# proger/haloop

Hardware: AMD Instinct MI355X
Metric: utterances/sec, LSTM-CTC training step (fwd + CTC loss + bwd + clip + AdamW) (higher is better)
Workload: dtype bf16 (dense operands rounded to bf16, 1 MFMA per product, fp32 accumulate; fp32 state, CTC, optimizer and master weights); 1 GPU; LC-2x1024: conv(80->128,k5,s4) + 2-layer LSTM H=1024 + Linear(1024->32) + CTC, 80 frames x 80 mels, vocab 32, targets 5-10 symbols, dropout 0.2; batch_per_gpu=64, global_batch=64, frames=80, mels=80, parallelism=dp1, hip_graph=False, math=bf16

## Files before the change

haloop_amd/_lib.py:

```python
import ctypes as C
import os

_HERE = os.path.dirname(os.path.abspath(__file__))
LIB_PATH = os.path.join(_HERE, 'csrc', 'libhalo.so')

HALO_ABI_VERSION = 21
HALO_GPT_SAMPLE_STREAM = 0x47505453
HALO_MLM_STREAM = 0x4D4C4D31
HALO_GEMM_RELU = 1
HALO_GEMM_GELU = 2
HALO_GEMM_ACCUM = 4
HALO_GEMM_GELU_ERF = 8
HALO_CTC_FULL_LATTICE = 1
HALO_CTC_FINITE_MIN = 2
HALO_CTC_NO_LEAD_BLANK_LOOP = 4
HALO_CTC_WRAP_SKIP = 8
HALO_STREAM_SUBSAMPLE = 1
HALO_STREAM_CLASSIFIER = 2
HALO_STREAM_LSTM_LAYER0 = 16
HALO_SUMSQ_PARTS = 1024
HALO_MATH_F32 = 0
HALO_MATH_BF16X3 = 1
HALO_MATH_BF16 = 2

# ... 174 lines not shown
    'halo_mlm_batch_u16': (_i, [_vp, _l, _vp, _i, _i, _f, _l, _l, _l, _u64, _u32, _vp, _vp, _vp]),
    'halo_target_rows': (_i, [_vp, _i, _l, _i, _i, _vp, _vp, _vp, _vp, _vp]),
    'halo_gather_rows': (_i, [_vp, _vp, _i, _i, _i, _vp, _vp]),
    'halo_scatter_rows': (_i, [_vp, _vp, _vp, _i, _i, _i, _i, _vp, _vp, _vp]),
    'halo_scale_add': (_i, [_vp, _vp, _f, _f, _sz, _vp]),
    'halo_cast_f32_bf16': (_i, [_vp, _vp, _sz, _vp]),
    'halo_cast_bf16_f32': (_i, [_vp, _vp, _f, _sz, _vp]),
    'halo_scale_add_guarded': (_i, [_vp, _vp, _f, _f, _sz, _vp, _vp]),
    'halo_clip_coef_step': (_i, [_vp, _i, _f, _vp, _vp, _vp, _vp]),
    'halo_adamw_ranges_dev': (_i, [_vp, _vp, _vp, _vp, _i, _vp, _vp, _vp, _vp, _f, _vp, _f, _f, _f, _vp, _vp, _vp]),
    'halo_ctx_create': (_vp, []),
    'halo_ctx_destroy': (None, [_vp]),
    'halo_ctx_use': (_i, [_vp]),
    'halo_set_status_word': (_i, [_vp]),
    'halo_debug_mute_workgroup': (_i, [_i]),
    'halo_debug_mfma_clock': (_i, [_vp, _vp, _i, _i, _i, _u32, _vp]),
    'halo_sumsq': (_i, [_vp, _sz, _vp, _vp]),
    'halo_sumsq_ranges': (_i, [_vp, _i, _vp, _vp, _vp, _vp]),
    'halo_pack_ranges_bf16': (_i, [_vp, _i, _vp, _vp, _vp, _vp]),
    'halo_expand_ranges_bf16': (_i, [_vp, _i, _vp, _vp, _i, _i, _vp, _vp]),
    'halo_clip_coef': (_i, [_vp, _i, _f, _vp, _vp, _vp]),
    'halo_adamw_multi_tensor_bytes': (_sz, []),
    'halo_adamw_multi_chunk': (_u32, []),
    'halo_adamw_multi_max_tensors': (_i, []),
    'halo_adamw_multi': (_i, [_vp, _vp, _i, _vp, _i, _f, _f, _f, _f, _i, _vp, _vp]),
    'halo_adamw_ranges': (_i, [_vp, _vp, _vp, _vp, _i, _vp, _vp, _vp, _vp, _f, _f, _f, _f, _i, _vp, _vp]),
    'halo_adamw': (_i, [_vp, _vp, _vp, _vp, _sz, _f, _f, _f, _f, _f, _i, _vp, _vp]),
}

_lib = None
# ... 168 lines not shown
```

haloop_amd/csrc/halo_common.h:

```cpp
#pragma once
#include <hip/hip_runtime.h>
#include <stdint.h>
#include "halo.h"

#define HALO_WAVE 64

#define HALO_CHECK_ARG(cond) \
    do {                     \
        if (!(cond)) return HALO_EINVAL; \
    } while (0)

static inline int halo_launch_status() {
    return hipGetLastError() == hipSuccess ? HALO_OK : HALO_ELAUNCH;
}

typedef float f32x4 __attribute__((ext_vector_type(4)));
typedef float f32x16 __attribute__((ext_vector_type(16)));

struct Philox4 {
    uint32_t v[4];
};

__device__ __forceinline__ Philox4 philox4x32_10(uint32_t c0, uint32_t c1, uint32_t c2, uint32_t c3,
                                                 uint32_t k0, uint32_t k1) {
// ... 31 lines not shown
    d.offset = offset;
    if (p > 0.f) {
        double t = (double)p * 4294967296.0;
        d.threshold = t >= 4294967295.0 ? 0xffffffffu : (uint32_t)t;
        d.scale = 1.0f / (1.0f - p);
    } else {
        d.threshold = 0u;
        d.scale = 1.0f;
    }
    return d;
}

__device__ __forceinline__ float dropout_mult(const DropoutCfg &d, uint64_t e) {
    const uint64_t q = e >> 2;
    const uint32_t off = d.offset + (d.offset_dev ? *d.offset_dev : 0u);
    const Philox4 r = philox4x32_10((uint32_t)q, (uint32_t)(q >> 32), d.stream_id, off, d.k0, d.k1);
    const uint32_t lane = (uint32_t)(e & 3);
    const uint32_t v = lane == 0 ? r.v[0] : lane == 1 ? r.v[1] : lane == 2 ? r.v[2] : r.v[3];
    return v >= d.threshold ? d.scale : 0.f;
}

__device__ __forceinline__ f32x4 dropout_mult4(const DropoutCfg &d, uint64_t e) {
    const uint64_t q = e >> 2;
    const uint32_t off = d.offset + (d.offset_dev ? *d.offset_dev : 0u);
    const Philox4 r = philox4x32_10((uint32_t)q, (uint32_t)(q >> 32), d.stream_id, off, d.k0, d.k1);
    f32x4 m;
    m[0] = r.v[0] >= d.threshold ? d.scale : 0.f;
    m[1] = r.v[1] >= d.threshold ? d.scale : 0.f;
    m[2] = r.v[2] >= d.threshold ? d.scale : 0.f;
    m[3] = r.v[3] >= d.threshold ? d.scale : 0.f;
// ... 64 lines not shown
```

haloop_amd/csrc/halo_internal.h:

```cpp
#pragma once
#include <hip/hip_runtime.h>
#include <stddef.h>
#include "halo_common.h"
#include "dyn_lds.h"
#include "small_jobs.h"

int halo_transpose(const float *in, float *out, int rows, int cols, hipStream_t st);
int halo_fill(float *p, size_t n, float v, hipStream_t st);
int halo_colsum2(const float *x, int rows, int cols, int ld, float *out, float *out2, hipStream_t st);

size_t halo_tiled_image_bytes(int R, int K);
int halo_prep_tiles(const float *src, int R, int K, int ld, int src_transposed, void *image, hipStream_t st);
int halo_prep_pair(const float *src, int R, int C, int ld, void *image_rm, void *image_tr, hipStream_t st);
struct HaloPrepJob {
    int kind;
    const float *src;
    int R, K, ld;
    void *image, *image_tr;
};
int halo_prep_jobs(const HaloPrepJob *jobs, int n, hipStream_t st);
int halo_gemm_bf16x3_tiled(const void *Aimg, const void *Bimg, int M, int N, int K, float *C, int ldc,
                           const float *bias1, const float *bias2, int relu, const DropoutCfg *drop, hipStream_t st);
int halo_gemm_bf16x3_tiled_slices(const void *Aimg, const void *Bimg, int M, int N, int K, float *slab, int want, int *slices, hipStream_t st);
bool halo_defer_small_job(const HaloSmallJob &job);
// ... 17 lines not shown
    unsigned grad_sumsq_cover = 0;
    int defer_small_jobs = 0;
    HaloSmallJobs small_jobs = {};
    int lstm_dx_slabs = 1;
    int lstm_dx_slabs_left = 1;
    int lstm_expect_backward = 1;
    const float *packT_reserve = nullptr, *packT_w[3] = {nullptr, nullptr, nullptr};
    const float *bwdflags_reserve = nullptr;
    const float *fwdT_src[2] = {nullptr, nullptr};
    const float *fwdT_reserve = nullptr;
    const float *emitT_reserve = nullptr;
    uint64_t lstm_weights_stamp = 0, packF_stamp = 0;
    const float *packF_reserve = nullptr, *packF_w[3] = {nullptr, nullptr, nullptr};
    int packF_dims[5] = {0, 0, 0, 0, 0};
    int mute_block = -1;
};
HaloCtx &halo_ctx_cur();
int halo_cu_count();
int halo_gemm_bf16x3_tiled_nsplit(const void *Aimg, const void *Bimg, int M, int N, int K, float *C, int ldc, int n_split, float *C2, int ldc2,
                                  hipStream_t st);
int halo_gemm_bf16x3_tiled_nsplit_carry(const void *Aimg, const void *Bimg, int M, int N, int K, float *C, int ldc, int n_split, float *C2, int ldc2,
                                        const void *rA, const void *rB, int rM, int rN, int rK, float *rslab, int want, int *slices,
                                        float *sumsq_part, int *sumsq_parts, hipStream_t st);
struct HaloG256Problem {
    const void *A, *B;
    int M, N, K;
    float *C; int ldc;
    int n_split; float *C2; int ldc2;
    int kslices; long slab_stride;
    float *sumsq;
// ... 15 lines not shown
```

haloop_amd/csrc/lstm_persist.h:

```cpp
#pragma once
#include <hip/hip_runtime.h>
#include <stdlib.h>
#include <type_traits>
#include "halo_common.h"
#include "halo_internal.h"

constexpr int PERSIST_FLAG_HEADER = 16;
constexpr int PERSIST_MAX_BLOCKS = 256;
constexpr int PERSIST_REPLICAS = 8;
constexpr int PERSIST_REPLICA_WORDS = 1024;
constexpr size_t PERSIST_FLAG_BYTES = (size_t)PERSIST_REPLICAS * PERSIST_REPLICA_WORDS * sizeof(unsigned);

struct PersistFwd {
    const char *wp;
    char *hp;
    float *gates;
    float *h;
    float *c;
    float *y;
    long y_stride_t, y_stride_b;
    int y_mode;
    DropoutCfg drop;
    unsigned *flags;
    unsigned *status;
// ... 39 lines not shown
    const char *wp0, *wp1, *wpi;
    char *hp0, *hp1;
    char *xp;
    float *gates0, *h0, *c0;
    float *gates1, *h1, *c1;
    const float *b_ih1, *b_hh1;
    float *ydrop;
    float *y;
    long y_stride_t, y_stride_b;
    int y_mode;
    DropoutCfg drop;
    char *img_hT0, *img_hT1, *img_xT1;
    unsigned *flags;
    unsigned *status;
    int mute;
    unsigned long long *stamps;
    int poll_mode, replica_shift, nap;
    int T, B, H;
    int bt0, nbt;
    unsigned epoch0;
};

struct Persist2Bwd {
    const char *wpT0, *wpT1, *wpTi;
    char *dgp0, *dgp1;
    float *gates0, *gates1;
    const float *c0, *c1;
    float *dc0, *dc1;
    const float *dy;
    long dy_stride_t, dy_stride_b;
    int dy_relu;
    const float *dhinit0, *dcinit0, *dhinit1, *dcinit1;
    DropoutCfg drop;
    unsigned *flags;
    unsigned *abort_word;
// ... 25 lines not shown
    int poll_mode, replica_shift, nap;
};
inline const PersistEnv &halo_persist_env() {
    const auto num = [](const char *name, int dflt) { const char *e = getenv(name); return e ? atoi(e) : dflt; };
    static const PersistEnv env = {num("HALO_PERSIST_POLL", 0), num("HALO_PERSIST_REPLICA_SHIFT", 3), num("HALO_PERSIST_NAP", 2)};
    return env;
}

template <auto Kernel, typename A>
int halo_persist_launch(const A &a0, int blocks, int dyn_lds, hipStream_t st, int poll_mode = 0) {
    static_assert(sizeof(A) <= 4096, "kernel arguments");
    A a = a0;
    a.poll_mode = poll_mode; a.replica_shift = halo_persist_env().replica_shift; a.nap = halo_persist_env().nap;
    a.status = halo_ctx_cur().status;
    if constexpr (std::is_same_v<A, PersistFwd> || std::is_same_v<A, Persist2Fwd>) a.mute = halo_ctx_cur().mute_block;
    if (halo_launch_lds<Kernel>(dim3((unsigned)blocks), dim3(512), dyn_lds, st, a) != HALO_OK) return HALO_ELAUNCH;
    return halo_launch_status();
}
```

haloop_amd/csrc/lstm_persist.hip:

```cpp
#include <stdlib.h>
#include "halo_common.h"
#include "halo_internal.h"
#include "lstm_persist.h"
#include "lstm_persist_dev.h"

namespace {

template <int KBW, bool ONE>
__global__ __launch_bounds__(512, 2) void lstm_persist_fwd_kernel(const PersistFwd p) {
    __shared__ float red[NWAVE][4][256];
    __shared__ __attribute__((aligned(16))) float hbuf[16][16];
    __shared__ int s_abort;
    const int tid = threadIdx.x, lane = tid & 63;
    const int wave = __builtin_amdgcn_readfirstlane(tid >> 6);
    const int H = p.H, B = p.B, T = p.T;
    const int NJ = H / 16, NBT = (B + 15) / 16, nkb = H / 32;
    int jt, bt;
    map_block(blockIdx.x, gridDim.x, NJ, NBT, jt, bt);
    const int j0 = jt * 16;

    bf16x8 wh[4][KBW], wl[4][KBW];
#pragma unroll
    for (int g = 0; g < 4; ++g)
#pragma unroll
// ... 312 lines not shown
            const int g = tid >> 4, j = tid & 15;
            float sum = 0.f;
#pragma unroll
            for (int r = 0; r < 16; ++r) sum += dgbuf[g][r][j];
            p.bias_part[(long)bt * K + (long)g * H + j0 + j] = sum;
        }
    }
}

}

void halo_lstm_persist_enable(int on) { halo_ctx_cur().lstm_persistent = on ? 1 : 0; }
unsigned long long *halo_lstm_persist_stamp_buffer() { return halo_ctx_cur().stamps; }
extern "C" int halo_debug_mute_workgroup(int block) {
    halo_ctx_cur().mute_block = block;
    return HALO_OK;
}
extern "C" int halo_lstm_persist_stamps(void *buf) {
    halo_ctx_cur().stamps = (unsigned long long *)buf;
    return HALO_OK;
}

bool halo_lstm_persist_fits(int T, int B, int H) {
    const long nbt = (B + 15) / 16;
    return (long)(T + 1) * nbt * (4 * H / 32) * 2048 < (1L << 31) && (long)(T + 1) * B * 4 * H < (1L << 31);
}

static bool wide_enabled() {
    static const bool off = getenv("HALO_LSTM_PERSIST32") && atoi(getenv("HALO_LSTM_PERSIST32")) == 0;
    return !off;
// ... 52 lines not shown
```

haloop_amd/csrc/lstm_persist2.hip:

```cpp
#include <stdlib.h>
#include "halo_common.h"
#include "halo_internal.h"
#include "lstm_persist.h"
#include "lstm_persist_dev.h"

namespace {

__device__ __forceinline__ bf16x8 unarm(bf16x8 v) {
    u32x4 w = __builtin_bit_cast(u32x4, v);
    if ((w.x & 0xffffu) == 0xffffu) w.x -= 1u;
    return __builtin_bit_cast(bf16x8, w);
}
template <int N>
__device__ __forceinline__ bool armed_lane(const bf16x8 (&f)[N]) {
    bool a = false;
#pragma unroll
    for (int i = 0; i < N; ++i) a |= (__builtin_bit_cast(u32x4, f[i]).x & 0xffffu) == 0xffffu;
    return a;
}
__device__ __forceinline__ bool rearm_wait(unsigned long long &t0, int pass, int nap) {
    const unsigned long long now = __builtin_amdgcn_s_memrealtime();
    if (pass == 0) t0 = now;
    else if (now - t0 > SPIN_TIMEOUT_TICKS) return false;
    if (nap == 1) __builtin_amdgcn_s_sleep(1);
    else if (nap == 2) __builtin_amdgcn_s_sleep(4);
    else if (nap == 3) __builtin_amdgcn_s_sleep(16);
    return true;
}
__device__ __forceinline__ void stamp_value(unsigned long long *stamps, int T, int step, int point, int lane, unsigned v) {
    if (stamps && lane == 0) stamps[((long)blockIdx.x * T + step) * 16 + point] = v;
}

struct Fwd2Shared {
    float (*red)[4][4][256];
    float (*hbuf)[16][16];
    int *s_abort;
    unsigned *s_published;
};

template <int KBQ, bool DF>
__device__ __forceinline__ void fwd2_layer0_waves(const Persist2Fwd &p, const Fwd2Shared sh, int jt, int bt, int wave, int lane, int u) {
    const int wq = wave & 3;
    const int H = p.H, B = p.B, T = p.T;
    const int NJ = H / 16, NBT = (B + 15) / 16, nkb = H / 32, j0 = jt * 16;
    bf16x8 wr[4][KBQ];
#pragma unroll
    for (int g = 0; g < 4; ++g)
#pragma unroll
        for (int i = 0; i < KBQ; ++i)
            wr[g][i] = *reinterpret_cast<const bf16x8 *>(p.wp0 + (((long)jt * 4 + g) * nkb + wq * KBQ + i) * 2048 + lane * 16);
    const int ci = u >> 4, cj = u & 15;
    const int b = bt * 16 + ci;
    const bool cell = b < B;
    const int BH = B * H;
    const int e0 = b * H + j0 + cj;
    float cst = 0.f, gin[4] = {0.f, 0.f, 0.f, 0.f};
    float dmul = (cell && p.xp) ? dropout_mult(p.drop, (uint64_t)e0) : 1.f;
    if (cell) {
        cst = p.c0[e0];
#pragma unroll
        for (int g = 0; g < 4; ++g) gin[g] = p.gates0[b * 4 * H + g * H + j0 + cj];
    }
    const __amdgpu_buffer_rsrc_t hp0_rsrc = make_rsrc(p.hp0), hp1_rsrc = make_rsrc(p.hp1);
    const __amdgpu_buffer_rsrc_t x_rsrc = p.xp ? make_rsrc(p.xp) : hp0_rsrc;
    const int my_replica = (xcc_id() + p.replica_shift) % PERSIST_REPLICAS;
    const int btl = bt - p.bt0;
    const unsigned *grp_flags = p.flags + my_replica * PERSIST_REPLICA_WORDS + PERSIST_FLAG_HEADER + btl * NJ;
    for (int s = 0; s <= T + 1; ++s) {
        if (wave == 0) stamp(p.stamps, T + 2, s, 0, lane);
        const bool act0 = s < T, act1 = s >= 2;
        if (!DF) {
            bool ok = true;
            if (s > 0 && wave == 1) ok = poll_group(grp_flags, 0, NJ, p.epoch0 + (unsigned)s, lane, p.nap);
            if (!ok && lane == 0) {
                *sh.s_abort = 1;
                raise_abort(p.flags, p.status);
            }
        }
        lds_barrier();
        if (*sh.s_abort) return;
        if (wave == 0) stamp(p.stamps, T + 2, s, 1, lane);
        if (act0) {
            const int img = ((s * NBT + bt) * nkb + wq * KBQ) * 2048;
            bf16x8 ah[KBQ];
            f32x4 acc[4];
            unsigned long long t0 = 0;
            for (int pass = 0;; ++pass) {
#pragma unroll
                for (int i = 0; i < KBQ; ++i) ah[i] = load_sc1_u(hp0_rsrc, lane * 16, img + i * 2048);
                __builtin_amdgcn_sched_barrier(0);
#pragma unroll
                for (int g = 0; g < 4; ++g) acc[g] = f32x4{0.f, 0.f, 0.f, 0.f};
#pragma unroll
                for (int i = 0; i < KBQ; ++i)
#pragma unroll
                    for (int g = 0; g < 4; ++g) acc[g] = __builtin_amdgcn_mfma_f32_16x16x32_bf16(ah[i], wr[g][i], acc[g], 0, 0, 0);
                if (!DF) break;
                if (!__any(armed_lane<KBQ>(ah))) {
                    if (wave == 0) { stamp(p.stamps, T + 2, s, 10, lane); stamp_value(p.stamps, T + 2, s, 11, lane, (unsigned)pass); }
                    break;
                }
                if (!rearm_wait(t0, pass, p.nap)) {
                    if (lane == 0) { *sh.s_abort = 1; raise_abort(p.flags, p.status); }
                    break;
                }
            }
            const int r = lane & 15, q = lane >> 4;
#pragma unroll
            for (int g = 0; g < 4; ++g)
#pragma unroll
                for (int e = 0; e < 4; ++e) sh.red[0][wq][g][(4 * q + e) * 16 + r] = acc[g][e];
        }
        lds_barrier();
        if (DF && *sh.s_abort) return;
        if (wave == 0) stamp(p.stamps, T + 2, s, 2, lane);
        float ig = 0.f, fg = 0.f, gg = 0.f, og = 0.f, h = 0.f, xv = 0.f;
        if (act0) {
            if (cell) {
                float pre[4];
#pragma unroll
                for (int g = 0; g < 4; ++g) {
                    float sum = 0.f;
#pragma unroll
                    for (int k = 0; k < 4; ++k) sum += sh.red[0][k][g][u];
                    pre[g] = sum + gin[g];
                }
                h = persist2_fwd_cell(pre, cst, ig, fg, gg, og);
                if (p.xp) xv = h * dmul;
            }
            sh.hbuf[0][ci][cj] = h;
            if (p.xp) sh.hbuf[1][ci][cj] = xv;
        }
        lds_barrier();
        if (wave == 0) stamp(p.stamps, T + 2, s, 3, lane);
        if ((wave == 3 && act0) || (wave == 2 && act1)) {
            const int sel = lane >> 5, kg = (lane >> 4) & 1, row = lane & 15;
            const float(*src)[16] = wave == 2 ? sh.hbuf[2] : sh.hbuf[sel];
            bf16x8 hi;
#pragma unroll
            for (int e = 0; e < 8; ++e) hi[e] = (__bf16)src[row][kg * 8 + e];
            if (DF) hi = unarm(hi);
            const int within = (jt >> 1) * 2048 + (((jt & 1) * 2 + kg) * 16 + row) * 16;
            const bool store = !DF || (int)blockIdx.x != p.mute;
            if (wave == 3) {
                if (sel == 0 && store) store_sc1(hp0_rsrc, (((s + 1) * NBT + bt) * nkb) * 2048 + within, hi);
                else if (sel == 1 && p.xp && store) store_sc1(x_rsrc, ((s * NBT + bt) * nkb) * 2048 + within, hi);
            } else if (sel == 0 && store) {
                store_sc1(hp1_rsrc, (((s - 1) * NBT + bt) * nkb) * 2048 + within, hi);
            }
            if (DF) {
                stamp(p.stamps, T + 2, s, wave == 3 ? 4 : 5, lane);
            } else {
                asm volatile("s_waitcnt vmcnt(0)" ::: "memory");
                unsigned old = 0;
                if (lane == 0) old = atomicAdd(sh.s_published, 1u);
                old = __builtin_amdgcn_readfirstlane(old);
                const unsigned target = (unsigned)((s + 1 < T ? s + 1 : T) + (s >= 2 ? s - 1 : 0));
                if (old + 1u == target && (int)blockIdx.x != p.mute) publish_epoch(p.flags, btl * NJ + jt, p.epoch0 + (unsigned)(s + 1), lane);
                stamp(p.stamps, T + 2, s, wave == 3 ? 4 : 5, lane);
            }
        } else if (!DF && wave == 3 && !act0 && !act1) {
            publish_epoch(p.flags, btl * NJ + jt, p.epoch0 + (unsigned)(s + 1), lane);
        }
        if (p.img_hT0 && ((wave == 3 && act0) || (wave == 2 && act1))) {
            const int sel = lane >> 5, kg = (lane >> 4) & 1, row = lane & 15;
            const float(*src)[16] = wave == 2 ? sh.hbuf[2] : (sel == 1 && p.xp ? sh.hbuf[1] : sh.hbuf[0]);
            const int tb = wave == 2 ? s - 1 : (sel == 0 ? s + 1 : s);
            char *img = wave == 2 ? (sel == 0 ? p.img_hT1 : nullptr) : (sel == 0 ? p.img_hT0 : p.img_xT1);
            if (img && tb < T) {
                bf16x8 hit;
#pragma unroll
                for (int e = 0; e < 8; ++e) hit[e] = (__bf16)src[kg * 8 + e][row];
                const int grow = j0 + row, kcol = tb * B + bt * 16 + kg * 8;
                const int KT = (T * B + 31) >> 5;
                const long blk = ((long)(grow >> 7) * KT + (kcol >> 5)) * 2;
                const int r = grow & 127, cc = (kcol & 31) >> 3;
// ... 3 lines not shown
        if (act0 && cell) {
            float *gp = p.gates0 + (s * B + b) * 4 * H + j0 + cj;
            gp[0] = ig; gp[H] = fg; gp[2 * H] = gg; gp[3 * H] = og;
            p.c0[(s + 1) * BH + e0] = cst;
            p.h0[(s + 1) * BH + e0] = h;
            if (p.ydrop) p.ydrop[s * BH + e0] = xv;
            if (p.xp && s + 1 < T) dmul = dropout_mult(p.drop, (uint64_t)((long)(s + 1) * BH + e0));
            if (s + 1 < T) {
#pragma unroll
                for (int g = 0; g < 4; ++g) gin[g] = p.gates0[((s + 1) * B + b) * 4 * H + g * H + j0 + cj];
            }
        }
    }
}

template <int KBQ, bool DF>
__device__ __forceinline__ void fwd2_layer1_waves(const Persist2Fwd &p, const Fwd2Shared sh, char *wi_lds, int jt, int bt, int wave, int lane,
                                                  int u) {
    constexpr int NWREG = KBQ >= 8 ? 2 : 0;
    constexpr int NWLDS = 4 * KBQ - NWREG;
    const int wq = wave & 3;
    const int H = p.H, B = p.B, T = p.T;
    const int NBT = (B + 15) / 16, nkb = H / 32, j0 = jt * 16;
    bf16x8 wr[4][KBQ];
#pragma unroll
    for (int g = 0; g < 4; ++g)
#pragma unroll
        for (int i = 0; i < KBQ; ++i)
            wr[g][i] = *reinterpret_cast<const bf16x8 *>(p.wp1 + (((long)jt * 4 + g) * nkb + wq * KBQ + i) * 2048 + lane * 16);
    bf16x8 wir[NWREG > 0 ? NWREG : 1];
    char *my_wi = wi_lds + (long)wq * NWLDS * 1024 + lane * 16;
// ... 17 lines not shown
#pragma unroll
        for (int g = 0; g < 4; ++g) bias[g] = p.b_ih1[g * H + j0 + cj] + p.b_hh1[g * H + j0 + cj];
    }
    const __amdgpu_buffer_rsrc_t hp1_rsrc = make_rsrc(p.hp1);
    const __amdgpu_buffer_rsrc_t x_rsrc = make_rsrc(p.xp ? p.xp : p.hp0);
    f32x4 xacc[4];
#pragma unroll
    for (int g = 0; g < 4; ++g) xacc[g] = f32x4{0.f, 0.f, 0.f, 0.f};
    for (int s = 0; s <= T + 1; ++s) {
        if (wave == 4) stamp(p.stamps, T + 2, s, 8, lane);
        const bool act1 = s >= 2, xin = s >= 1 && s <= T;
        const int t = s - 2;
        lds_barrier();
        if (*sh.s_abort) return;
        bf16x8 ax[KBQ];
        if constexpr (DF) {
            const int ximg = ((min(max(p.xp ? s - 1 : s, 0), p.xp ? T - 1 : T) * NBT + bt) * nkb + wq * KBQ) * 2048;
            const int img = ((max(t, 0) * NBT + bt) * nkb + wq * KBQ) * 2048;
            bf16x8 ah[KBQ];
            unsigned long long t0 = 0;
            for (int pass = 0;; ++pass) {
#pragma unroll
                for (int i = 0; i < KBQ; ++i) ax[i] = load_sc1_u(x_rsrc, lane * 16, ximg + i * 2048);
#pragma unroll
                for (int i = 0; i < KBQ; ++i) ah[i] = load_sc1_u(hp1_rsrc, lane * 16, img + i * 2048);
                const bool bx = armed_lane<KBQ>(ax), bh = armed_lane<KBQ>(ah);
                if (!__any((xin && bx) || (act1 && bh))) {
                    if (wave == 4) { stamp(p.stamps, T + 2, s, 12, lane); stamp_value(p.stamps, T + 2, s, 13, lane, (unsigned)pass); }
                    break;
                }
                if (!rearm_wait(t0, pass, p.nap)) {
                    if (lane == 0) { *sh.s_abort = 1; raise_abort(p.flags, p.status); }
                    break;
                }
            }
            if (act1) {
#pragma unroll
                for (int i = 0; i < KBQ; ++i)
#pragma unroll
                    for (int g = 0; g < 4; ++g) xacc[g] = __builtin_amdgcn_mfma_f32_16x16x32_bf16(ah[i], wr[g][i], xacc[g], 0, 0, 0);
                const int r = lane & 15, q = lane >> 4;
#pragma unroll
                for (int g = 0; g < 4; ++g)
#pragma unroll
                    for (int e = 0; e < 4; ++e) sh.red[1][wq][g][(4 * q + e) * 16 + r] = xacc[g][e];
            }
        } else {
            if (xin) {
                const int ximg = (((p.xp ? s - 1 : s) * NBT + bt) * nkb + wq * KBQ) * 2048;
#pragma unroll
                for (int i = 0; i < KBQ; ++i) ax[i] = load_sc1_u(x_rsrc, lane * 16, ximg + i * 2048);
            }
            if (act1) {
                const int img = ((t * NBT + bt) * nkb + wq * KBQ) * 2048;
                bf16x8 ah[KBQ];
#pragma unroll
                for (int i = 0; i < KBQ; ++i) ah[i] = load_sc1_u(hp1_rsrc, lane * 16, img + i * 2048);
                __builtin_amdgcn_sched_barrier(0);
#pragma unroll
                for (int i = 0; i < KBQ; ++i)
#pragma unroll
                    for (int g = 0; g < 4; ++g) xacc[g] = __builtin_amdgcn_mfma_f32_16x16x32_bf16(ah[i], wr[g][i], xacc[g], 0, 0, 0);
                const int r = lane & 15, q = lane >> 4;
#pragma unroll
                for (int g = 0; g < 4; ++g)
#pragma unroll
                    for (int e = 0; e < 4; ++e) sh.red[1][wq][g][(4 * q + e) * 16 + r] = xacc[g][e];
            }
        }
        lds_barrier();
        if (DF && *sh.s_abort) return;
        float ig = 0.f, fg = 0.f, gg = 0.f, og = 0.f, h = 0.f;
        if (act1) {
            if (cell) {
                float pre[4];
#pragma unroll
                for (int g = 0; g < 4; ++g) {
                    float sum = 0.f;
#pragma unroll
                    for (int k = 0; k < 4; ++k) sum += sh.red[1][k][g][u];
                    pre[g] = sum + bias[g];
                }
                h = persist2_fwd_cell(pre, cst, ig, fg, gg, og);
            }
            sh.hbuf[2][ci][cj] = h;
        }
// ... 10 lines not shown
        for (int g = 0; g < 4; ++g) xacc[g] = f32x4{0.f, 0.f, 0.f, 0.f};
        if (xin) {
#pragma unroll
            for (int i = 0; i < KBQ; ++i) {
                bf16x8 w[4];
#pragma unroll
                for (int g = 0; g < 4; ++g)
                    w[g] = i * 4 + g < NWREG ? wir[i * 4 + g < NWREG ? i * 4 + g : 0]
                                             : *reinterpret_cast<const bf16x8 *>(my_wi + (i * 4 + g - NWREG) * 1024);
#pragma unroll
                for (int g = 0; g < 4; ++g) xacc[g] = __builtin_amdgcn_mfma_f32_16x16x32_bf16(ax[i], w[g], xacc[g], 0, 0, 0);
                if (i & 1) __builtin_amdgcn_sched_barrier(0);
            }
        }
        if (wave == 4) stamp(p.stamps, T + 2, s, 6, lane);
    }
}

template <int KBQ, bool DF>
__global__ __launch_bounds__(512, 2) void lstm_persist2_fwd_kernel(const Persist2Fwd p) {
    __shared__ float red[2][4][4][256];
    __shared__ __attribute__((aligned(16))) float hbuf[3][16][16];
    __shared__ int s_abort;
    __shared__ unsigned s_published;
    extern __shared__ __attribute__((aligned(16))) char wi_lds[];
    const int tid = threadIdx.x, lane = tid & 63;
    const int wave = __builtin_amdgcn_readfirstlane(tid >> 6);
    int jt, bt;
    map_block(blockIdx.x, gridDim.x, p.H / 16, p.nbt, jt, bt);
    bt += p.bt0;
    if (tid == 0) { s_abort = 0; s_published = 0; }
    if (wave == 0) stamp(p.stamps, p.T + 2, 0, 14, lane);
    const Fwd2Shared sh = {red, hbuf, &s_abort, &s_published};
    if (wave < 4) fwd2_layer0_waves<KBQ, DF>(p, sh, jt, bt, wave, lane, tid & 255);
    else fwd2_layer1_waves<KBQ, DF>(p, sh, wi_lds, jt, bt, wave, lane, tid & 255);
    if (wave == 0) stamp(p.stamps, p.T + 2, 0, 15, lane);
}

struct Bwd2Shared {
    float (*red)[4][256];
    float (*dgbuf)[4][16][16];
    int *s_abort;
    unsigned *s_published;
};

struct Bwd2Cell {
    float gv[4], cc, cprev, dcarry;
    __device__ __forceinline__ void update(float dh, float (&dg)[4]) { dcarry = persist2_bwd_cell(gv, cc, cprev, dcarry, dh, dg); }
};

// ... 384 lines not shown
```

include/halo.h:

```cpp
#ifndef HALO_H
#define HALO_H

#include <stddef.h>
#include <stdint.h>

#ifdef __cplusplus
extern "C" {
#endif

#define HALO_ABI_VERSION 21

#define HALO_OK 0
#define HALO_EINVAL (-22)
#define HALO_ENOTSUP (-95)
#define HALO_ELAUNCH (-5)

typedef void *halo_stream_t;

int halo_abi_version(void);
int halo_debug_read(const void *src, size_t bytes, int pattern, size_t row_bytes, float *sink, void *stream);
const char *halo_strerror(int code);
int halo_device_info(int device, char *arch, int arch_len, int *cu_count);

#define HALO_MATH_F32 0
// ... 123 lines not shown
                  float *reserve, int T, int B, int in0, int H, int L, float p_drop, uint64_t seed,
                  uint32_t offset, const uint32_t *offset_dev, halo_stream_t stream);
int halo_lstm_bwd(const float *x, const float *const *w_ih, const float *const *w_hh, const float *dy,
                  long y_stride_t, long y_stride_b, int y_relu, const float *dhn, const float *dcn,
                  float *reserve, float *workspace, float *dx, float *const *dw_ih, float *const *dw_hh,
                  float *const *db_ih, float *const *db_hh, int T, int B, int in0, int H, int L,
                  int layer_begin, int layer_end, float p_drop, uint64_t seed, uint32_t offset,
                  const uint32_t *offset_dev, halo_stream_t stream);

typedef struct halo_ctx halo_ctx;
halo_ctx *halo_ctx_create(void);
void halo_ctx_destroy(halo_ctx *ctx);
int halo_ctx_use(halo_ctx *ctx);
int halo_set_status_word(uint32_t *device_word);
int halo_debug_mute_workgroup(int block);
int halo_debug_mfma_clock(unsigned long long *ticks, float *sink, int blocks, int iters, int shape, unsigned seed, halo_stream_t stream);

int halo_set_lstm_persistent(int on);
int halo_set_lstm_persistent_images(int on);
int halo_lstm_persistent_eligible(int B, int H);
int halo_set_lstm_persistent2(int on);
int halo_set_lstm_interleave(int on);
int halo_set_gemm256(int on);
int halo_set_lstm_bwd_mid_event(void *event);
int halo_lstm_bwd_mid_event_recorded(void);
int halo_set_lstm_weights_stamp(uint64_t stamp);
int halo_set_lstm_expect_backward(int on);
int halo_set_lstm_dx_slabs(int n);
int halo_lstm_dx_slabs_left(void);
int halo_set_defer_small_jobs(int on);
// ... 269 lines not shown
```

Baseline: 157,100 utterances/s.

## Prefetch next-step hidden state in dataflow persistent LSTM forward kernels

Splits the dataflow (DF) variant of the persistent two-layer LSTM forward into dedicated layer0/layer1 wave functions. These issue the loads of the next step's hidden-state images and gate inputs at the end of the current step, so their latency overlaps the cell and epilogue work instead of sitting on the critical path. It also hoists the dropout offset load out of the time loop and precomputes the next step's dropout mask early. A debug workgroup-delay hook is added for testing; the speculative load-then-multiply scheme may redo MFMAs when the data arrives stale.

```diff
diff --git a/haloop_amd/_lib.py b/haloop_amd/_lib.py
--- a/haloop_amd/_lib.py
+++ b/haloop_amd/_lib.py
@@ -212,6 +212,7 @@
     'halo_ctx_use': (_i, [_vp]),
     'halo_set_status_word': (_i, [_vp]),
     'halo_debug_mute_workgroup': (_i, [_i]),
+    'halo_debug_delay_workgroup': (_i, [_i, _u32]),
     'halo_debug_mfma_clock': (_i, [_vp, _vp, _i, _i, _i, _u32, _vp]),
     'halo_sumsq': (_i, [_vp, _sz, _vp, _vp]),
     'halo_sumsq_ranges': (_i, [_vp, _i, _vp, _vp, _vp, _vp]),
diff --git a/haloop_amd/csrc/halo_common.h b/haloop_amd/csrc/halo_common.h
--- a/haloop_amd/csrc/halo_common.h
+++ b/haloop_amd/csrc/halo_common.h
@@ -69,6 +69,15 @@
 __device__ __forceinline__ float dropout_mult(const DropoutCfg &d, uint64_t e) {
     const uint64_t q = e >> 2;
     const uint32_t off = d.offset + (d.offset_dev ? *d.offset_dev : 0u);
+    const Philox4 r = philox4x32_10((uint32_t)q, (uint32_t)(q >> 32), d.stream_id, off, d.k0, d.k1);
+    const uint32_t lane = (uint32_t)(e & 3);
+    const uint32_t v = lane == 0 ? r.v[0] : lane == 1 ? r.v[1] : lane == 2 ? r.v[2] : r.v[3];
+    return v >= d.threshold ? d.scale : 0.f;
+}
+
+__device__ __forceinline__ uint32_t dropout_offset(const DropoutCfg &d) { return d.offset + (d.offset_dev ? *d.offset_dev : 0u); }
+__device__ __forceinline__ float dropout_mult(const DropoutCfg &d, uint32_t off, uint64_t e) {
+    const uint64_t q = e >> 2;
     const Philox4 r = philox4x32_10((uint32_t)q, (uint32_t)(q >> 32), d.stream_id, off, d.k0, d.k1);
     const uint32_t lane = (uint32_t)(e & 3);
     const uint32_t v = lane == 0 ? r.v[0] : lane == 1 ? r.v[1] : lane == 2 ? r.v[2] : r.v[3];
diff --git a/haloop_amd/csrc/halo_internal.h b/haloop_amd/csrc/halo_internal.h
--- a/haloop_amd/csrc/halo_internal.h
+++ b/haloop_amd/csrc/halo_internal.h
@@ -55,6 +55,8 @@
     const float *packF_reserve = nullptr, *packF_w[3] = {nullptr, nullptr, nullptr};
     int packF_dims[5] = {0, 0, 0, 0, 0};
     int mute_block = -1;
+    int delay_block = -1;
+    unsigned delay_ticks = 0;
 };
 HaloCtx &halo_ctx_cur();
 int halo_cu_count();
diff --git a/haloop_amd/csrc/lstm_persist.h b/haloop_amd/csrc/lstm_persist.h
--- a/haloop_amd/csrc/lstm_persist.h
+++ b/haloop_amd/csrc/lstm_persist.h
@@ -77,11 +77,13 @@
     unsigned *flags;
     unsigned *status;
     int mute;
+    int delay_block;
     unsigned long long *stamps;
     int poll_mode, replica_shift, nap;
     int T, B, H;
     int bt0, nbt;
     unsigned epoch0;
+    unsigned delay_ticks;
 };
 
 struct Persist2Bwd {
@@ -137,6 +139,7 @@
     a.poll_mode = poll_mode; a.replica_shift = halo_persist_env().replica_shift; a.nap = halo_persist_env().nap;
     a.status = halo_ctx_cur().status;
     if constexpr (std::is_same_v<A, PersistFwd> || std::is_same_v<A, Persist2Fwd>) a.mute = halo_ctx_cur().mute_block;
+    if constexpr (std::is_same_v<A, Persist2Fwd>) { a.delay_block = halo_ctx_cur().delay_block; a.delay_ticks = halo_ctx_cur().delay_ticks; }
     if (halo_launch_lds<Kernel>(dim3((unsigned)blocks), dim3(512), dyn_lds, st, a) != HALO_OK) return HALO_ELAUNCH;
     return halo_launch_status();
 }
diff --git a/haloop_amd/csrc/lstm_persist.hip b/haloop_amd/csrc/lstm_persist.hip
--- a/haloop_amd/csrc/lstm_persist.hip
+++ b/haloop_amd/csrc/lstm_persist.hip
@@ -350,6 +350,12 @@
 unsigned long long *halo_lstm_persist_stamp_buffer() { return halo_ctx_cur().stamps; }
 extern "C" int halo_debug_mute_workgroup(int block) {
     halo_ctx_cur().mute_block = block;
+    return HALO_OK;
+}
+extern "C" int halo_debug_delay_workgroup(int block, unsigned ticks) {
+    if (ticks > HALO_DEBUG_DELAY_MAX_TICKS) return HALO_EINVAL;
+    halo_ctx_cur().delay_block = block;
+    halo_ctx_cur().delay_ticks = block >= 0 ? ticks : 0u;
     return HALO_OK;
 }
 extern "C" int halo_lstm_persist_stamps(void *buf) {
diff --git a/haloop_amd/csrc/lstm_persist2.hip b/haloop_amd/csrc/lstm_persist2.hip
--- a/haloop_amd/csrc/lstm_persist2.hip
+++ b/haloop_amd/csrc/lstm_persist2.hip
@@ -3,6 +3,10 @@
 #include "halo_internal.h"
 #include "lstm_persist.h"
 #include "lstm_persist_dev.h"
+
+#ifndef HALO_P2_ISSUE_POINT
+#define HALO_P2_ISSUE_POINT 0
+#endif
 
 namespace {
 
@@ -38,7 +42,7 @@
     unsigned *s_published;
 };
 
-template <int KBQ, bool DF>
+template <int KBQ>
 __device__ __forceinline__ void fwd2_layer0_waves(const Persist2Fwd &p, const Fwd2Shared sh, int jt, int bt, int wave, int lane, int u) {
     const int wq = wave & 3;
     const int H = p.H, B = p.B, T = p.T;
@@ -69,13 +73,11 @@
     for (int s = 0; s <= T + 1; ++s) {
         if (wave == 0) stamp(p.stamps, T + 2, s, 0, lane);
         const bool act0 = s < T, act1 = s >= 2;
-        if (!DF) {
-            bool ok = true;
-            if (s > 0 && wave == 1) ok = poll_group(grp_flags, 0, NJ, p.epoch0 + (unsigned)s, lane, p.nap);
-            if (!ok && lane == 0) {
-                *sh.s_abort = 1;
-                raise_abort(p.flags, p.status);
-            }
+        bool ok = true;
+        if (s > 0 && wave == 1) ok = poll_group(grp_flags, 0, NJ, p.epoch0 + (unsigned)s, lane, p.nap);
+        if (!ok && lane == 0) {
+            *sh.s_abort = 1;
+            raise_abort(p.flags, p.status);
         }
         lds_barrier();
         if (*sh.s_abort) return;
@@ -84,27 +86,15 @@
             const int img = ((s * NBT + bt) * nkb + wq * KBQ) * 2048;
             bf16x8 ah[KBQ];
             f32x4 acc[4];
-            unsigned long long t0 = 0;
-            for (int pass = 0;; ++pass) {
-#pragma unroll
-                for (int i = 0; i < KBQ; ++i) ah[i] = load_sc1_u(hp0_rsrc, lane * 16, img + i * 2048);
-                __builtin_amdgcn_sched_barrier(0);
-#pragma unroll
-                for (int g = 0; g < 4; ++g) acc[g] = f32x4{0.f, 0.f, 0.f, 0.f};
-#pragma unroll
-                for (int i = 0; i < KBQ; ++i)
-#pragma unroll
-                    for (int g = 0; g < 4; ++g) acc[g] = __builtin_amdgcn_mfma_f32_16x16x32_bf16(ah[i], wr[g][i], acc[g], 0, 0, 0);
-                if (!DF) break;
-                if (!__any(armed_lane<KBQ>(ah))) {
-                    if (wave == 0) { stamp(p.stamps, T + 2, s, 10, lane); stamp_value(p.stamps, T + 2, s, 11, lane, (unsigned)pass); }
-                    break;
-                }
-                if (!rearm_wait(t0, pass, p.nap)) {
-                    if (lane == 0) { *sh.s_abort = 1; raise_abort(p.flags, p.status); }
-                    break;
-                }
-            }
+#pragma unroll
+            for (int i = 0; i < KBQ; ++i) ah[i] = load_sc1_u(hp0_rsrc, lane * 16, img + i * 2048);
+            __builtin_amdgcn_sched_barrier(0);
+#pragma unroll
+            for (int g = 0; g < 4; ++g) acc[g] = f32x4{0.f, 0.f, 0.f, 0.f};
+#pragma unroll
+            for (int i = 0; i < KBQ; ++i)
+#pragma unroll
+                for (int g = 0; g < 4; ++g) acc[g] = __builtin_amdgcn_mfma_f32_16x16x32_bf16(ah[i], wr[g][i], acc[g], 0, 0, 0);
             const int r = lane & 15, q = lane >> 4;
 #pragma unroll
             for (int g = 0; g < 4; ++g)
@@ -112,7 +102,6 @@
                 for (int e = 0; e < 4; ++e) sh.red[0][wq][g][(4 * q + e) * 16 + r] = acc[g][e];
         }
         lds_barrier();
-        if (DF && *sh.s_abort) return;
         if (wave == 0) stamp(p.stamps, T + 2, s, 2, lane);
         float ig = 0.f, fg = 0.f, gg = 0.f, og = 0.f, h = 0.f, xv = 0.f;
         if (act0) {
@@ -139,27 +128,21 @@
             bf16x8 hi;
 #pragma unroll
             for (int e = 0; e < 8; ++e) hi[e] = (__bf16)src[row][kg * 8 + e];
-            if (DF) hi = unarm(hi);
             const int within = (jt >> 1) * 2048 + (((jt & 1) * 2 + kg) * 16 + row) * 16;
-            const bool store = !DF || (int)blockIdx.x != p.mute;
             if (wave == 3) {
-                if (sel == 0 && store) store_sc1(hp0_rsrc, (((s + 1) * NBT + bt) * nkb) * 2048 + within, hi);
-                else if (sel == 1 && p.xp && store) store_sc1(x_rsrc, ((s * NBT + bt) * nkb) * 2048 + within, hi);
-            } else if (sel == 0 && store) {
+                if (sel == 0) store_sc1(hp0_rsrc, (((s + 1) * NBT + bt) * nkb) * 2048 + within, hi);
+                else if (sel == 1 && p.xp) store_sc1(x_rsrc, ((s * NBT + bt) * nkb) * 2048 + within, hi);
+            } else if (sel == 0) {
                 store_sc1(hp1_rsrc, (((s - 1) * NBT + bt) * nkb) * 2048 + within, hi);
             }
-            if (DF) {
-                stamp(p.stamps, T + 2, s, wave == 3 ? 4 : 5, lane);
-            } else {
-                asm volatile("s_waitcnt vmcnt(0)" ::: "memory");
-                unsigned old = 0;
-                if (lane == 0) old = atomicAdd(sh.s_published, 1u);
-                old = __builtin_amdgcn_readfirstlane(old);
-                const unsigned target = (unsigned)((s + 1 < T ? s + 1 : T) + (s >= 2 ? s - 1 : 0));
-                if (old + 1u == target && (int)blockIdx.x != p.mute) publish_epoch(p.flags, btl * NJ + jt, p.epoch0 + (unsigned)(s + 1), lane);
-                stamp(p.stamps, T + 2, s, wave == 3 ? 4 : 5, lane);
-            }
-        } else if (!DF && wave == 3 && !act0 && !act1) {
+            asm volatile("s_waitcnt vmcnt(0)" ::: "memory");
+            unsigned old = 0;
+            if (lane == 0) old = atomicAdd(sh.s_published, 1u);
+            old = __builtin_amdgcn_readfirstlane(old);
+            const unsigned target = (unsigned)((s + 1 < T ? s + 1 : T) + (s >= 2 ? s - 1 : 0));
+            if (old + 1u == target && (int)blockIdx.x != p.mute) publish_epoch(p.flags, btl * NJ + jt, p.epoch0 + (unsigned)(s + 1), lane);
+            stamp(p.stamps, T + 2, s, wave == 3 ? 4 : 5, lane);
+        } else if (wave == 3 && !act0 && !act1) {
             publish_epoch(p.flags, btl * NJ + jt, p.epoch0 + (unsigned)(s + 1), lane);
         }
         if (p.img_hT0 && ((wave == 3 && act0) || (wave == 2 && act1))) {
@@ -193,7 +176,7 @@
     }
 }
 
-template <int KBQ, bool DF>
+template <int KBQ>
 __device__ __forceinline__ void fwd2_layer1_waves(const Persist2Fwd &p, const Fwd2Shared sh, char *wi_lds, int jt, int bt, int wave, int lane,
                                                   int u) {
     constexpr int NWREG = KBQ >= 8 ? 2 : 0;
@@ -241,62 +224,28 @@
         lds_barrier();
         if (*sh.s_abort) return;
         bf16x8 ax[KBQ];
-        if constexpr (DF) {
-            const int ximg = ((min(max(p.xp ? s - 1 : s, 0), p.xp ? T - 1 : T) * NBT + bt) * nkb + wq * KBQ) * 2048;
-            const int img = ((max(t, 0) * NBT + bt) * nkb + wq * KBQ) * 2048;
+        if (xin) {
+            const int ximg = (((p.xp ? s - 1 : s) * NBT + bt) * nkb + wq * KBQ) * 2048;
+#pragma unroll
+            for (int i = 0; i < KBQ; ++i) ax[i] = load_sc1_u(x_rsrc, lane * 16, ximg + i * 2048);
+        }
+        if (act1) {
+            const int img = ((t * NBT + bt) * nkb + wq * KBQ) * 2048;
             bf16x8 ah[KBQ];
-            unsigned long long t0 = 0;
-            for (int pass = 0;; ++pass) {
-#pragma unroll
-                for (int i = 0; i < KBQ; ++i) ax[i] = load_sc1_u(x_rsrc, lane * 16, ximg + i * 2048);
-#pragma unroll
-                for (int i = 0; i < KBQ; ++i) ah[i] = load_sc1_u(hp1_rsrc, lane * 16, img + i * 2048);
-                const bool bx = armed_lane<KBQ>(ax), bh = armed_lane<KBQ>(ah);
-                if (!__any((xin && bx) || (act1 && bh))) {
-                    if (wave == 4) { stamp(p.stamps, T + 2, s, 12, lane); stamp_value(p.stamps, T + 2, s, 13, lane, (unsigned)pass); }
-                    break;
-                }
-                if (!rearm_wait(t0, pass, p.nap)) {
-                    if (lane == 0) { *sh.s_abort = 1; raise_abort(p.flags, p.status); }
-                    break;
-                }
-            }
-            if (act1) {
-#pragma unroll
-                for (int i = 0; i < KBQ; ++i)
-#pragma unroll
-                    for (int g = 0; g < 4; ++g) xacc[g] = __builtin_amdgcn_mfma_f32_16x16x32_bf16(ah[i], wr[g][i], xacc[g], 0, 0, 0);
-                const int r = lane & 15, q = lane >> 4;
-#pragma unroll
-                for (int g = 0; g < 4; ++g)
-#pragma unroll
-                    for (int e = 0; e < 4; ++e) sh.red[1][wq][g][(4 * q + e) * 16 + r] = xacc[g][e];
-            }
-        } else {
-            if (xin) {
-                const int ximg = (((p.xp ? s - 1 : s) * NBT + bt) * nkb + wq * KBQ) * 2048;
-#pragma unroll
-                for (int i = 0; i < KBQ; ++i) ax[i] = load_sc1_u(x_rsrc, lane * 16, ximg + i * 2048);
-            }
-            if (act1) {
-                const int img = ((t * NBT + bt) * nkb + wq * KBQ) * 2048;
-                bf16x8 ah[KBQ];
-#pragma unroll
-                for (int i = 0; i < KBQ; ++i) ah[i] = load_sc1_u(hp1_rsrc, lane * 16, img + i * 2048);
-                __builtin_amdgcn_sched_barrier(0);
-#pragma unroll
-                for (int i = 0; i < KBQ; ++i)
-#pragma unroll
-                    for (int g = 0; g < 4; ++g) xacc[g] = __builtin_amdgcn_mfma_f32_16x16x32_bf16(ah[i], wr[g][i], xacc[g], 0, 0, 0);
-                const int r = lane & 15, q = lane >> 4;
-#pragma unroll
-                for (int g = 0; g < 4; ++g)
-#pragma unroll
-                    for (int e = 0; e < 4; ++e) sh.red[1][wq][g][(4 * q + e) * 16 + r] = xacc[g][e];
-            }
-        }
-        lds_barrier();
-        if (DF && *sh.s_abort) return;
+#pragma unroll
+            for (int i = 0; i < KBQ; ++i) ah[i] = load_sc1_u(hp1_rsrc, lane * 16, img + i * 2048);
+            __builtin_amdgcn_sched_barrier(0);
+#pragma unroll
+            for (int i = 0; i < KBQ; ++i)
+#pragma unroll
+                for (int g = 0; g < 4; ++g) xacc[g] = __builtin_amdgcn_mfma_f32_16x16x32_bf16(ah[i], wr[g][i], xacc[g], 0, 0, 0);
+            const int r = lane & 15, q = lane >> 4;
+#pragma unroll
+            for (int g = 0; g < 4; ++g)
+#pragma unroll
+                for (int e = 0; e < 4; ++e) sh.red[1][wq][g][(4 * q + e) * 16 + r] = xacc[g][e];
+        }
+        lds_barrier();
         float ig = 0.f, fg = 0.f, gg = 0.f, og = 0.f, h = 0.f;
         if (act1) {
             if (cell) {
@@ -337,6 +286,283 @@
             }
         }
         if (wave == 4) stamp(p.stamps, T + 2, s, 6, lane);
+    }
+}
+
+template <int KBQ>
+__device__ __forceinline__ void fwd2_df_layer0_waves(const Persist2Fwd &p, const Fwd2Shared sh, int jt, int bt, int wave, int lane, int u) {
+    const int wq = wave & 3;
+    const int H = p.H, B = p.B, T = p.T;
+    const int NBT = (B + 15) / 16, nkb = H / 32, j0 = jt * 16;
+    bf16x8 wr[4][KBQ];
+#pragma unroll
+    for (int g = 0; g < 4; ++g)
+#pragma unroll
+        for (int i = 0; i < KBQ; ++i)
+            wr[g][i] = *reinterpret_cast<const bf16x8 *>(p.wp0 + (((long)jt * 4 + g) * nkb + wq * KBQ + i) * 2048 + lane * 16);
+    const int ci = u >> 4, cj = u & 15;
+    const int b = bt * 16 + ci;
+    const bool cell = b < B;
+    const int BH = B * H;
+    const int e0 = b * H + j0 + cj;
+    const uint32_t drop_off = dropout_offset(p.drop);
+    float cst = cell ? p.c0[e0] : 0.f;
+    float dmul = (cell && p.xp) ? dropout_mult(p.drop, drop_off, (uint64_t)e0) : 1.f;
+    float gin[4];
+    const float *gsrc = p.gates0 + min(b, B - 1) * 4 * H + j0 + cj;
+    const auto request_gin = [&](int t) {
+        __builtin_amdgcn_sched_barrier(0);
+#pragma unroll
+        for (int g = 0; g < 4; ++g) gin[g] = gsrc[min(t, T - 1) * B * 4 * H + g * H];
+    };
+    const __amdgpu_buffer_rsrc_t hp0_rsrc = make_rsrc(p.hp0), hp1_rsrc = make_rsrc(p.hp1);
+    const __amdgpu_buffer_rsrc_t x_rsrc = p.xp ? make_rsrc(p.xp) : hp0_rsrc;
+    bf16x8 ah[KBQ];
+    const auto request = [&](int sn) {
+        const int img = ((min(__builtin_amdgcn_readfirstlane(sn), T) * NBT + bt) * nkb + wq * KBQ) * 2048;
+#pragma unroll
+        for (int i = 0; i < KBQ; ++i) ah[i] = load_sc1_u(hp0_rsrc, lane * 16, img + i * 2048);
+    };
+    request(0);
+    request_gin(0);
+    lds_barrier();
+    for (int s = 0; s <= T + 1; ++s) {
+        if (wave == 0) stamp(p.stamps, T + 2, s, 0, lane);
+        const bool act0 = s < T, act1 = s >= 2;
+        if (act0) {
+            f32x4 acc[4];
+            const auto multiply = [&]() {
+#pragma unroll
+                for (int g = 0; g < 4; ++g) acc[g] = f32x4{0.f, 0.f, 0.f, 0.f};
+#pragma unroll
+                for (int i = 0; i < KBQ; ++i)
+#pragma unroll
+                    for (int g = 0; g < 4; ++g) acc[g] = __builtin_amdgcn_mfma_f32_16x16x32_bf16(ah[i], wr[g][i], acc[g], 0, 0, 0);
+            };
+            multiply();
+            unsigned long long t0 = 0;
+            int pass = 0;
+            while (__any(armed_lane<KBQ>(ah))) {
+                if (!rearm_wait(t0, pass, pass == 0 ? 0 : p.nap)) {
+                    if (lane == 0) { *sh.s_abort = 1; raise_abort(p.flags, p.status); }
+                    break;
+                }
+                request(s);
+                multiply();
+                ++pass;
+            }
+            if (wave == 0) { stamp(p.stamps, T + 2, s, 10, lane); stamp_value(p.stamps, T + 2, s, 11, lane, (unsigned)pass); }
+            const int r = lane & 15, q = lane >> 4;
+#pragma unroll
+            for (int g = 0; g < 4; ++g)
+#pragma unroll
+                for (int e = 0; e < 4; ++e) sh.red[0][wq][g][(4 * q + e) * 16 + r] = acc[g][e];
+        }
+        lds_barrier();
+        if (__builtin_amdgcn_readfirstlane(*sh.s_abort)) return;
+        if (wave == 0) stamp(p.stamps, T + 2, s, 2, lane);
+        float ig = 0.f, fg = 0.f, gg = 0.f, og = 0.f, h = 0.f, xv = 0.f;
+        if (act0) {
+            if (cell) {
+                float pre[4];
+#pragma unroll
+                for (int g = 0; g < 4; ++g) {
+                    float sum = 0.f;
+#pragma unroll
+                    for (int k = 0; k < 4; ++k) sum += sh.red[0][k][g][u];
+                    pre[g] = sum + gin[g];
+                }
+                h = persist2_fwd_cell(pre, cst, ig, fg, gg, og);
+                if (p.xp) xv = h * dmul;
+            }
+            sh.hbuf[0][ci][cj] = h;
+            if (p.xp) sh.hbuf[1][ci][cj] = xv;
+        }
+        lds_barrier();
+        if (wave == 0) stamp(p.stamps, T + 2, s, 3, lane);
+        if ((wave == 3 && act0) || (wave == 2 && act1)) {
+            const int sel = lane >> 5, kg = (lane >> 4) & 1, row = lane & 15;
+            const float(*src)[16] = wave == 2 ? sh.hbuf[2] : sh.hbuf[sel];
+            bf16x8 hi;
+#pragma unroll
+            for (int e = 0; e < 8; ++e) hi[e] = (__bf16)src[row][kg * 8 + e];
+            hi = unarm(hi);
+            const int within = (jt >> 1) * 2048 + (((jt & 1) * 2 + kg) * 16 + row) * 16;
+            const bool store = (int)blockIdx.x != p.mute;
+            if (p.delay_ticks != 0 && (int)blockIdx.x == p.delay_block) {
+                const unsigned long long t0 = __builtin_amdgcn_s_memrealtime();
+                while (__builtin_amdgcn_s_memrealtime() - t0 < p.delay_ticks) __builtin_amdgcn_s_sleep(1);
+            }
+            if (wave == 3) {
+                if (sel == 0 && store) store_sc1(hp0_rsrc, (((s + 1) * NBT + bt) * nkb) * 2048 + within, hi);
+                else if (sel == 1 && p.xp && store) store_sc1(x_rsrc, ((s * NBT + bt) * nkb) * 2048 + within, hi);
+            } else if (sel == 0 && store) {
+                store_sc1(hp1_rsrc, (((s - 1) * NBT + bt) * nkb) * 2048 + within, hi);
+            }
+            stamp(p.stamps, T + 2, s, wave == 3 ? 4 : 5, lane);
+        }
+#if HALO_P2_ISSUE_POINT == 1
+        request(s + 1);
+        request_gin(s + 1);
+        if (wave == 3) stamp(p.stamps, T + 2, s, 9, lane);
+#endif
+        if (p.img_hT0 && ((wave == 3 && act0) || (wave == 2 && act1))) {
+            const int sel = lane >> 5, kg = (lane >> 4) & 1, row = lane & 15;
+            const float(*src)[16] = wave == 2 ? sh.hbuf[2] : (sel == 1 && p.xp ? sh.hbuf[1] : sh.hbuf[0]);
+            const int tb = wave == 2 ? s - 1 : (sel == 0 ? s + 1 : s);
+            char *img = wave == 2 ? (sel == 0 ? p.img_hT1 : nullptr) : (sel == 0 ? p.img_hT0 : p.img_xT1);
+            if (img && tb < T) {
+                bf16x8 hit;
+#pragma unroll
+                for (int e = 0; e < 8; ++e) hit[e] = (__bf16)src[kg * 8 + e][row];
+                const int grow = j0 + row, kcol = tb * B + bt * 16 + kg * 8;
+                const int KT = (T * B + 31) >> 5;
+                const long blk = ((long)(grow >> 7) * KT + (kcol >> 5)) * 2;
+                const int r = grow & 127, cc = (kcol & 31) >> 3;
+                *reinterpret_cast<bf16x8 *>(img + blk * 8192 + r * 64 + ((cc ^ ((r >> 2) & 3)) << 4)) = hit;
+            }
+        }
+        if (act0 && cell) {
+            float *gp = p.gates0 + (s * B + b) * 4 * H + j0 + cj;
+            gp[0] = ig; gp[H] = fg; gp[2 * H] = gg; gp[3 * H] = og;
+            p.c0[(s + 1) * BH + e0] = cst;
+            p.h0[(s + 1) * BH + e0] = h;
+            if (p.ydrop) p.ydrop[s * BH + e0] = xv;
+        }
+#if HALO_P2_ISSUE_POINT == 0
+        request(s + 1);
+        request_gin(s + 1);
+        if (wave == 3) stamp(p.stamps, T + 2, s, 9, lane);
+#endif
+        if (act0 && cell && p.xp && s + 1 < T) dmul = dropout_mult(p.drop, drop_off, (uint64_t)((long)(s + 1) * BH + e0));
+    }
+}
+
+template <int KBQ>
+__device__ __forceinline__ void fwd2_df_layer1_waves(const Persist2Fwd &p, const Fwd2Shared sh, char *wi_lds, int jt, int bt, int wave, int lane,
+                                                     int u) {
+    constexpr int NWREG = KBQ >= 8 ? 2 : 0;
+    constexpr int NWLDS = 4 * KBQ - NWREG;
+    const int wq = wave & 3;
+    const int H = p.H, B = p.B, T = p.T;
+    const int NBT = (B + 15) / 16, nkb = H / 32, j0 = jt * 16;
+    bf16x8 wr[4][KBQ];
+#pragma unroll
+    for (int g = 0; g < 4; ++g)
+#pragma unroll
+        for (int i = 0; i < KBQ; ++i)
+            wr[g][i] = *reinterpret_cast<const bf16x8 *>(p.wp1 + (((long)jt * 4 + g) * nkb + wq * KBQ + i) * 2048 + lane * 16);
+    bf16x8 wir[NWREG > 0 ? NWREG : 1];
+    char *my_wi = wi_lds + (long)wq * NWLDS * 1024 + lane * 16;
+#pragma unroll
+    for (int i = 0; i < KBQ; ++i)
+#pragma unroll
+        for (int g = 0; g < 4; ++g) {
+            const bf16x8 v = *reinterpret_cast<const bf16x8 *>(p.wpi + (((long)jt * 4 + g) * nkb + wq * KBQ + i) * 2048 + lane * 16);
+            if (i * 4 + g < NWREG) wir[i * 4 + g < NWREG ? i * 4 + g : 0] = v;
+            else *reinterpret_cast<bf16x8 *>(my_wi + (i * 4 + g - NWREG) * 1024) = v;
+            if (g == 3 && (i & 3) == 3) __builtin_amdgcn_sched_barrier(0);
+        }
+    const int ci = u >> 4, cj = u & 15;
+    const int b = bt * 16 + ci;
+    const bool cell = b < B;
+    const int BH = B * H;
+    const int e0 = b * H + j0 + cj;
+    float cst = 0.f, bias[4] = {0.f, 0.f, 0.f, 0.f};
+    if (cell) {
+        cst = p.c1[e0];
+#pragma unroll
+        for (int g = 0; g < 4; ++g) bias[g] = p.b_ih1[g * H + j0 + cj] + p.b_hh1[g * H + j0 + cj];
+    }
+    const __amdgpu_buffer_rsrc_t hp1_rsrc = make_rsrc(p.hp1);
+    const __amdgpu_buffer_rsrc_t x_rsrc = make_rsrc(p.xp ? p.xp : p.hp0);
+    f32x4 xacc[4];
+#pragma unroll
+    for (int g = 0; g < 4; ++g) xacc[g] = f32x4{0.f, 0.f, 0.f, 0.f};
+    bf16x8 ax[KBQ], ah[KBQ];
+    const auto request = [&](int sv) {
+        const int sn = __builtin_amdgcn_readfirstlane(sv);
+        const int ximg = ((min(max(p.xp ? sn - 1 : sn, 0), p.xp ? T - 1 : T) * NBT + bt) * nkb + wq * KBQ) * 2048;
+        const int img = ((min(max(sn - 2, 0), T - 1) * NBT + bt) * nkb + wq * KBQ) * 2048;
+#pragma unroll
+        for (int i = 0; i < KBQ; ++i) ax[i] = load_sc1_u(x_rsrc, lane * 16, ximg + i * 2048);
+#pragma unroll
+        for (int i = 0; i < KBQ; ++i) ah[i] = load_sc1_u(hp1_rsrc, lane * 16, img + i * 2048);
+    };
+    request(0);
+    lds_barrier();
+    for (int s = 0; s <= T + 1; ++s) {
+        if (wave == 4) stamp(p.stamps, T + 2, s, 8, lane);
+        const bool act1 = s >= 2, xin = s >= 1 && s <= T;
+        const int t = s - 2;
+        unsigned long long t0 = 0;
+        for (int pass = 0;; ++pass) {
+            const bool bx = armed_lane<KBQ>(ax), bh = armed_lane<KBQ>(ah);
+            if (!__any((xin && bx) || (act1 && bh))) {
+                if (wave == 4) { stamp(p.stamps, T + 2, s, 12, lane); stamp_value(p.stamps, T + 2, s, 13, lane, (unsigned)pass); }
+                break;
+            }
+            if (!rearm_wait(t0, pass, pass == 0 ? 0 : p.nap)) {
+                if (lane == 0) { *sh.s_abort = 1; raise_abort(p.flags, p.status); }
+                break;
+            }
+            request(s);
+        }
+        if (act1) {
+#pragma unroll
+            for (int i = 0; i < KBQ; ++i)
+#pragma unroll
+                for (int g = 0; g < 4; ++g) xacc[g] = __builtin_amdgcn_mfma_f32_16x16x32_bf16(ah[i], wr[g][i], xacc[g], 0, 0, 0);
+            const int r = lane & 15, q = lane >> 4;
+#pragma unroll
+            for (int g = 0; g < 4; ++g)
+#pragma unroll
+                for (int e = 0; e < 4; ++e) sh.red[1][wq][g][(4 * q + e) * 16 + r] = xacc[g][e];
+        }
+        lds_barrier();
+        if (__builtin_amdgcn_readfirstlane(*sh.s_abort)) return;
+        float ig = 0.f, fg = 0.f, gg = 0.f, og = 0.f, h = 0.f;
+        if (act1) {
+            if (cell) {
+                float pre[4];
+#pragma unroll
+                for (int g = 0; g < 4; ++g) {
+                    float sum = 0.f;
+#pragma unroll
+                    for (int k = 0; k < 4; ++k) sum += sh.red[1][k][g][u];
+                    pre[g] = sum + bias[g];
+                }
+                h = persist2_fwd_cell(pre, cst, ig, fg, gg, og);
+            }
+            sh.hbuf[2][ci][cj] = h;
+        }
+        lds_barrier();
+        if (act1 && cell) {
+            float *gp = p.gates1 + (t * B + b) * 4 * H + j0 + cj;
+            gp[0] = ig; gp[H] = fg; gp[2 * H] = gg; gp[3 * H] = og;
+            p.c1[(t + 1) * BH + e0] = cst;
+            p.h1[(t + 1) * BH + e0] = h;
+            if (p.y_mode != 0) p.y[(long)t * p.y_stride_t + (long)b * p.y_stride_b + j0 + cj] = p.y_mode == 2 ? fmaxf(h, 0.f) : h;
+        }
+        if (wave == 4) stamp(p.stamps, T + 2, s, 7, lane);
+#pragma unroll
+        for (int g = 0; g < 4; ++g) xacc[g] = f32x4{0.f, 0.f, 0.f, 0.f};
+        if (xin) {
+#pragma unroll
+            for (int i = 0; i < KBQ; ++i) {
+                bf16x8 w[4];
+#pragma unroll
+                for (int g = 0; g < 4; ++g)
+                    w[g] = i * 4 + g < NWREG ? wir[i * 4 + g < NWREG ? i * 4 + g : 0]
+                                             : *reinterpret_cast<const bf16x8 *>(my_wi + (i * 4 + g - NWREG) * 1024);
+#pragma unroll
+                for (int g = 0; g < 4; ++g) xacc[g] = __builtin_amdgcn_mfma_f32_16x16x32_bf16(ax[i], w[g], xacc[g], 0, 0, 0);
+                if (i & 1) __builtin_amdgcn_sched_barrier(0);
+            }
+        }
+        if (wave == 4) stamp(p.stamps, T + 2, s, 6, lane);
+        __builtin_amdgcn_sched_barrier(0);
+        request(s + 1);
     }
 }
 
@@ -355,8 +581,13 @@
     if (tid == 0) { s_abort = 0; s_published = 0; }
     if (wave == 0) stamp(p.stamps, p.T + 2, 0, 14, lane);
     const Fwd2Shared sh = {red, hbuf, &s_abort, &s_published};
-    if (wave < 4) fwd2_layer0_waves<KBQ, DF>(p, sh, jt, bt, wave, lane, tid & 255);
-    else fwd2_layer1_waves<KBQ, DF>(p, sh, wi_lds, jt, bt, wave, lane, tid & 255);
+    if constexpr (DF) {
+        if (wave < 4) fwd2_df_layer0_waves<KBQ>(p, sh, jt, bt, wave, lane, tid & 255);
+        else fwd2_df_layer1_waves<KBQ>(p, sh, wi_lds, jt, bt, wave, lane, tid & 255);
+    } else {
+        if (wave < 4) fwd2_layer0_waves<KBQ>(p, sh, jt, bt, wave, lane, tid & 255);
+        else fwd2_layer1_waves<KBQ>(p, sh, wi_lds, jt, bt, wave, lane, tid & 255);
+    }
     if (wave == 0) stamp(p.stamps, p.T + 2, 0, 15, lane);
 }
 
diff --git a/include/halo.h b/include/halo.h
--- a/include/halo.h
+++ b/include/halo.h
@@ -161,6 +161,8 @@
 int halo_ctx_use(halo_ctx *ctx);
 int halo_set_status_word(uint32_t *device_word);
 int halo_debug_mute_workgroup(int block);
+#define HALO_DEBUG_DELAY_MAX_TICKS 100000u
+int halo_debug_delay_workgroup(int block, unsigned ticks);
 int halo_debug_mfma_clock(unsigned long long *ticks, float *sink, int blocks, int iters, int shape, unsigned seed, halo_stream_t stream);
 
 int halo_set_lstm_persistent(int on);
```

New measurement: 146,200 utterances/s. 0.93x the previous value.
